# shz9/viprs

Measured on AMD Instinct MI355X. Metric: SNP-updates/sec/E-step (1M SNPs, ~1700 LD blocks), higher is better.
Workload: dtype f32

## Files before the change

### viprs_amd/csrc/estep_grid_mfma.h

```cpp
#pragma once
#include "device_math.h"
#include "kernels_common.h"

namespace viprs {

#ifdef VIPRS_GRID_PROFILE
#define GPROF(slot, cond) do { if (blk == 0 && lane == 0 && p < 32 && (cond)) s_prof[p][slot] = (unsigned)wall_clock64(); } while (0)
#else
#define GPROF(slot, cond) do { } while (0)
#endif

constexpr int kGridIoPitch = kPanel + 1;
constexpr int kGridIoArr = kGridModels * kGridIoPitch;
constexpr int kGridIoFloats = 4 * kGridIoArr;
constexpr int kGridAFloats = kPanel * kGridModels;
constexpr int kGridDiagFloats = kPanel * kPanel;
constexpr int kGridCarryFloats = (kPanel + 32) * 64;
constexpr int kGridQxPitch = kPanel + 4;
constexpr int kGridQxFloats = kGridModels * kGridQxPitch;
constexpr int kGridLdsFloats = 2 * kGridIoFloats + 2 * kGridAFloats + 2 * kGridDiagFloats + kGridCarryFloats + 2 * kGridQxFloats;

using f32x16 = __attribute__((ext_vector_type(16))) float;
using f32x4 = __attribute__((ext_vector_type(4))) float;
using f32x2 = __attribute__((ext_vector_type(2))) float;


template <typename U>
__device__ __forceinline__ void tile_load_rows(float (&R)[kPanel], const U* __restrict__ base, int stride, int b,
                                               int rp, int ct, int lane) {
    const int row0 = rp * kPanel;
    const int last_row = min(kPanel, b - row0) - 1;
    const U* __restrict__ p = base + (int64_t)row0 * stride + ct * kPanel + lane;
#pragma unroll
    for (int k = 0; k < kPanel; ++k) R[k] = static_cast<float>(p[(int64_t)min(k, last_row) * stride]);
    asm volatile("" ::: "memory");
}

template <bool SCALED = false>
__device__ __forceinline__ void tile_compute(f32x16& acc0, f32x16& acc1, const float (&R)[kPanel],
                                             const float* __restrict__ a_lds, int lane, float scale = 1.0f) {
    const int half = lane >> 5, l31 = lane & 31;
#pragma unroll
    for (int kr = 0; kr < kPanel; kr += 2) {
        auto sw = __builtin_amdgcn_permlane32_swap(__float_as_uint(R[kr]), __float_as_uint(R[kr + 1]), false, false);
        const float b0 = __uint_as_float(sw[0]), b1 = __uint_as_float(sw[1]);
        const float a_raw = a_lds[(kr + half) * kGridModels + l31];
        const float aop = SCALED ? scale * a_raw : a_raw;
        acc0 = __builtin_amdgcn_mfma_f32_32x32x2f32(aop, b0, acc0, 0, 0, 0);
        acc1 = __builtin_amdgcn_mfma_f32_32x32x2f32(aop, b1, acc1, 0, 0, 0);
    }
}

template <typename U> struct Vec4 { typedef U type __attribute__((ext_vector_type(4))); };
typedef float f32x4u __attribute__((ext_vector_type(4), aligned(4)));

template <bool FULL>
__device__ __forceinline__ void wtile_load_acc_issue(f32x16 (&acc)[4], const EStepArgs<float>& A, const int* act, int64_t s0,
                                                     int b, int c0, bool lane_ok, int lane) {
    const int half = lane >> 5, c = c0 + 4 * (lane & 31);
#pragma unroll
    for (int r = 0; r < 16; ++r) {
        const int g = (r & 3) + 8 * (r >> 2) + 4 * half;
        const unsigned off = (unsigned)act[g] * (unsigned)A.m + (unsigned)s0;
        if (FULL) {
            const f32x4u v = *reinterpret_cast<const f32x4u*>(A.q + off + (lane_ok ? c : 0));
#pragma unroll
            for (int j = 0; j < 4; ++j) acc[j][r] = v[j];
        } else {
#pragma unroll
            for (int j = 0; j < 4; ++j) acc[j][r] = A.q[off + ((lane_ok && c + j < b) ? c + j : 0)];
        }
    }
    asm volatile("" ::: "memory");
}
template <bool FULL>
__device__ __forceinline__ void wtile_load_acc_finish(f32x16 (&acc)[4], int b, int c0, bool lane_ok, int n_models, int lane) {
    const int half = lane >> 5, c = c0 + 4 * (lane & 31);
#pragma unroll
    for (int r = 0; r < 16; ++r) {
        const int g = (r & 3) + 8 * (r >> 2) + 4 * half;
        const bool ok = lane_ok && g < n_models;
#pragma unroll
        for (int j = 0; j < 4; ++j) acc[j][r] = (ok && (FULL || c + j < b)) ? acc[j][r] : 0.0f;
    }
}
template <bool FULL>
__device__ __forceinline__ void wtile_load_acc(f32x16 (&acc)[4], const EStepArgs<float>& A, const int* act, int64_t s0,
                                               int b, int c0, bool lane_ok, int n_models, int lane) {
    wtile_load_acc_issue<FULL>(acc, A, act, s0, b, c0, lane_ok, lane);
    wtile_load_acc_finish<FULL>(acc, b, c0, lane_ok, n_models, lane);
}

template <bool FULL>
__device__ __forceinline__ void wtile_store_acc(const f32x16 (&acc)[4], const EStepArgs<float>& A, const int* act,
                                                int64_t s0, int b, int c0, bool lane_ok, int n_models, int lane) {
    const int half = lane >> 5, c = c0 + 4 * (lane & 31);
#pragma unroll
    for (int r = 0; r < 16; ++r) {
        const int g = (r & 3) + 8 * (r >> 2) + 4 * half;
        if (lane_ok && g < n_models) {
            const unsigned off = (unsigned)act[g] * (unsigned)A.m + (unsigned)s0 + c;
            if (FULL) {
                *reinterpret_cast<f32x4u*>(A.q + off) = f32x4u{acc[0][r], acc[1][r], acc[2][r], acc[3][r]};
            } else {
#pragma unroll
                for (int j = 0; j < 4; ++j)
                    if (c + j < b) A.q[off + j] = acc[j][r];
            }
        }
    }
}

template <bool FULL>
__device__ __forceinline__ void wtile_add_to_q(const f32x16 (&acc)[4], const EStepArgs<float>& A, const int* act, int64_t s0,
                                               int b, int c0, bool lane_ok, int n_models, int lane, float dq) {
    const int half = lane >> 5, c = c0 + 4 * (lane & 31);
#pragma unroll
    for (int r = 0; r < 16; ++r) {
        const int g = (r & 3) + 8 * (r >> 2) + 4 * half;
        if (lane_ok && g < n_models) {
            const unsigned off = (unsigned)act[g] * (unsigned)A.m + (unsigned)s0 + c;
            if (FULL) {
                const f32x4u v = *reinterpret_cast<const f32x4u*>(A.q + off);
                *reinterpret_cast<f32x4u*>(A.q + off) =
                    f32x4u{v[0] + dq * acc[0][r], v[1] + dq * acc[1][r], v[2] + dq * acc[2][r], v[3] + dq * acc[3][r]};
            } else {
#pragma unroll
                for (int j = 0; j < 4; ++j)
                    if (c + j < b) A.q[off + j] = A.q[off + j] + dq * acc[j][r];
            }
        }
    }
}

template <bool SYM, bool EXACT = true, bool STORE_D = false>
__device__ __forceinline__ void grid_chain_panel(const EStepArgs<float>& A, float* io, float* la, float* dg, float* qx, int p, int b,
                                                 int64_t s0, int lane, int n_models, float dq, const ExpTab& tab
#ifdef VIPRS_GRID_PROFILE
                                                 , int blk, unsigned* prof
#endif
                                                 ) {
    const int cg = lane & 31, ch = lane >> 5;
    const bool has_model = cg < n_models;
#ifdef VIPRS_GRID_PROFILE
    unsigned (*s_prof)[12] = reinterpret_cast<unsigned (*)[12]>(prof);
#endif
    const int r0 = p * kPanel;
    const int nrows = min(kPanel, b - r0);
    float* iob = io + (p & 1) * kGridIoFloats + cg * kGridIoPitch;
    float* lap = la + (p & 1) * kGridAFloats + cg;
    const float* drow = dg + (p & 1) * kGridDiagFloats + 32 * ch;
    float* qmine = qx + (p & 1) * kGridQxFloats + cg * kGridQxPitch + 32 * ch;
    f32x2 qv[16];
#pragma unroll
    for (int i = 0; i < 8; ++i) {
        const f32x4 v = *reinterpret_cast<const f32x4*>(qmine + 4 * i);
        qv[2 * i] = has_model ? f32x2{v[0], v[1]} : f32x2{0.0f, 0.0f};
        qv[2 * i + 1] = has_model ? f32x2{v[2], v[3]} : f32x2{0.0f, 0.0f};
    }
    const float betav = A.std_beta[s0 + min(r0 + lane, b - 1)];
#ifdef VIPRS_GRID_PROFILE
    asm volatile("s_waitcnt vmcnt(0) lgkmcnt(0)" ::: "memory");
#endif
    GPROF(2, true);
    f32x2 rw[16];
    auto load_row = [&](f32x2 (&dst)[16], int jr, int g4) {
        const float* rp = drow + jr * kPanel;
        const int o0 = 16 * (g4 & 1), o1 = 16 * ((g4 + 1) & 1);
#pragma unroll
        for (int i = 0; i < 4; ++i) {
            const f32x4 x = *reinterpret_cast<const f32x4*>(rp + o0 + 4 * i);
            const f32x4 y = *reinterpret_cast<const f32x4*>(rp + o1 + 4 * i);
            dst[2 * i] = f32x2{x[0], x[1]};
            dst[2 * i + 1] = f32x2{x[2], x[3]};
            dst[8 + 2 * i] = f32x2{y[0], y[1]};
            dst[8 + 2 * i + 1] = f32x2{y[2], y[3]};
        }
    };
    load_row(rw, 0, 0);
    float mm = iob[0 * kGridIoArr], ulog = iob[1 * kGridIoArr], hvt = iob[2 * kGridIoArr],
          eta_old = iob[3 * kGridIoArr];
#pragma unroll 1
    for (int g4 = 0; g4 < kPanel / 16; ++g4) {
        const bool hi_owner = g4 >= 2;
        const bool owner = (ch == 1) == hi_owner;
        float* const iog = iob + 16 * g4;
        float* const lag = lap + 16 * g4 * kGridModels;
#pragma unroll
        for (int k = 0; k < 16; ++k) {
            const int jj = 16 * g4 + k;
            const bool live = jj < nrows;
            const int jn = min(jj + 1, kPanel - 1);
            const int kn = (k < 15) ? k + 1 : ((g4 < kPanel / 16 - 1) ? 16 : 15);
            const float mm_n = iog[0 * kGridIoArr + kn], ulog_n = iog[1 * kGridIoArr + kn],
                        hvt_n = iog[2 * kGridIoArr + kn], eta_n = iog[3 * kGridIoArr + kn];
            const unsigned qbits = __float_as_uint(qv[k >> 1][k & 1]);
            auto sw = __builtin_amdgcn_permlane32_swap(qbits, qbits, false, false);
            const float qcur = __uint_as_float(hi_owner ? sw[1] : sw[0]);
            const float beta = __builtin_bit_cast(float, __builtin_amdgcn_readlane(__builtin_bit_cast(int, betav), jj));
            const float mu = mm * (beta - qcur);
            const float u = ulog + hvt * mu * mu;
            const float gamma = EXACT ? sigmoid_exact<kLookupPerLane>(u, tab) : sigmoid_fast(u);
            const float d = gamma * mu - eta_old;
            const float a = (live && has_model) ? dq * d : 0.0f;
            f32x2 rn[16];
            load_row(rn, jn, (jj + 1) >> 4);
            const f32x2 a2 = {a, a};
#pragma unroll
            for (int c = 0; c < 16; ++c) {
                qv[c] = __builtin_elementwise_fma(rw[c], a2, qv[c]);
                asm volatile("" : "+v"(qv[c]));
            }
            if (SYM) qv[k >> 1][k & 1] -= (live && owner && has_model) ? d : 0.0f;
            iog[0 * kGridIoArr + k] = mu;
            iog[1 * kGridIoArr + k] = gamma;
            iog[2 * kGridIoArr + k] = d;
            iog[3 * kGridIoArr + k] = eta_old + d;
            lag[k * kGridModels] = STORE_D ? ((live && has_model) ? d : 0.0f) : a;
            mm = mm_n; ulog = ulog_n; hvt = hvt_n; eta_old = eta_n;
#pragma unroll
            for (int c = 0; c < 16; ++c) rw[c] = rn[c];
            __builtin_amdgcn_sched_barrier(0);
        }
#pragma unroll
        for (int c = 0; c < 8; ++c) {
            const f32x2 t = qv[c];
            qv[c] = qv[8 + c];
            qv[8 + c] = t;
        }
    }
    GPROF(3, true);
    if (has_model) {
#pragma unroll
        for (int i = 0; i < 8; ++i)
            *reinterpret_cast<f32x4*>(qmine + 4 * i) = f32x4{qv[2 * i][0], qv[2 * i][1], qv[2 * i + 1][0], qv[2 * i + 1][1]};
    }
}

template <bool SYM, bool EXACT = true>
__device__ __forceinline__ void grid_chain_panel_mfma(const EStepArgs<float>& A, float* io, float* la, float* dg, float* qx, int p,
                                                      int b, int64_t s0, int lane, int n_models, float dq, const ExpTab& tab) {
    const int cg = lane & 31, ch = lane >> 5;
    const bool has_model = cg < n_models;
    const int r0 = p * kPanel;
    const int nrows = min(kPanel, b - r0);
    float* iob = io + (p & 1) * kGridIoFloats + cg * kGridIoPitch;
    float* lap = la + (p & 1) * kGridAFloats + cg;
    const float* drow = dg + (p & 1) * kGridDiagFloats + lane;
    float* qm = qx + (p & 1) * kGridQxFloats + cg * kGridQxPitch;
    f32x16 acc0, acc1;
#pragma unroll
    for (int g = 0; g < 4; ++g) {
        const f32x4 v = *reinterpret_cast<const f32x4*>(qm + 8 * g + 4 * ch);
        const f32x4 w = *reinterpret_cast<const f32x4*>(qm + 32 + 8 * g + 4 * ch);
#pragma unroll
        for (int e = 0; e < 4; ++e) {
            acc0[4 * g + e] = has_model ? v[e] : 0.0f;
            acc1[4 * g + e] = has_model ? w[e] : 0.0f;
        }
    }
    const float betav = A.std_beta[s0 + min(r0 + lane, b - 1)];
    float mm = iob[0 * kGridIoArr], ulog = iob[1 * kGridIoArr], hvt = iob[2 * kGridIoArr], eta_old = iob[3 * kGridIoArr];
    float rowv = drow[0];
    float qcur;
    {
        const unsigned x = __float_as_uint(acc0[0]);
        auto sx = __builtin_amdgcn_permlane32_swap(x, x, false, false);
        qcur = __uint_as_float(sx[0]);
    }
#pragma unroll
    for (int jj = 0; jj < kPanel; ++jj) {
        const bool live = jj < nrows;
        const int jn = (jj + 1 < kPanel) ? jj + 1 : jj;
        const float mm_n = iob[0 * kGridIoArr + jn], ulog_n = iob[1 * kGridIoArr + jn], hvt_n = iob[2 * kGridIoArr + jn],
                    eta_n = iob[3 * kGridIoArr + jn];
        const float rowv_n = drow[jn * kPanel];
        const float beta = __builtin_bit_cast(float, __builtin_amdgcn_readlane(__builtin_bit_cast(int, betav), jj));
        const float mu = mm * (beta - qcur);
        const float u = ulog + hvt * mu * mu;
        const float gamma = EXACT ? sigmoid_exact<kLookupPerLane>(u, tab) : sigmoid_fast(u);
        const float d = gamma * mu - eta_old;
        const float a = (live && has_model) ? dq * d : 0.0f;
        const float dsub = (SYM && live && has_model) ? d : 0.0f;
        __builtin_amdgcn_sched_barrier(0);
        auto sr = __builtin_amdgcn_permlane32_swap(__float_as_uint(rowv), __float_as_uint(rowv), false, false);
        const float row_lo = __uint_as_float(sr[0]), row_hi = __uint_as_float(sr[1]);
        const float A0 = ch ? ((SYM && cg == jj) ? -1.0f : 0.0f) : row_lo;
        const float A1 = ch ? ((SYM && cg + 32 == jj) ? -1.0f : 0.0f) : row_hi;
        const float B = ch ? dsub : a;
        float qnext = 0.0f;
        if (jj + 1 < kPanel) {
            constexpr int kDummy = 0; (void)kDummy;
            const int c1 = jj + 1, i1 = c1 & 31, r1 = (i1 & 3) + 4 * (i1 >> 3), h1 = (i1 >> 2) & 1;
            const unsigned x = __float_as_uint((c1 >> 5) ? acc1[r1] : acc0[r1]);
            auto sx = __builtin_amdgcn_permlane32_swap(x, x, false, false);
            const float xq = __uint_as_float(h1 ? sx[1] : sx[0]);
            const float dn = __builtin_bit_cast(float, __builtin_amdgcn_readlane(__builtin_bit_cast(int, rowv), c1));
            qnext = __builtin_fmaf(dn, a, xq);
        }
        acc0 = __builtin_amdgcn_mfma_f32_32x32x2f32(A0, B, acc0, 0, 0, 0);
        acc1 = __builtin_amdgcn_mfma_f32_32x32x2f32(A1, B, acc1, 0, 0, 0);
        if (has_model && live && ch == 0) {
            iob[0 * kGridIoArr + jj] = mu;
            iob[1 * kGridIoArr + jj] = gamma;
            iob[2 * kGridIoArr + jj] = d;
            iob[3 * kGridIoArr + jj] = eta_old + d;
        }
        if (ch == 0) lap[jj * kGridModels] = a;
        mm = mm_n; ulog = ulog_n; hvt = hvt_n; eta_old = eta_n; rowv = rowv_n; qcur = qnext;
        __builtin_amdgcn_sched_barrier(0);
    }
    if (has_model) {
#pragma unroll
        for (int g = 0; g < 4; ++g) {
            *reinterpret_cast<f32x4*>(qm + 8 * g + 4 * ch) = f32x4{acc0[4 * g], acc0[4 * g + 1], acc0[4 * g + 2], acc0[4 * g + 3]};
            *reinterpret_cast<f32x4*>(qm + 32 + 8 * g + 4 * ch) = f32x4{acc1[4 * g], acc1[4 * g + 1], acc1[4 * g + 2], acc1[4 * g + 3]};
        }
    }
}

constexpr int kGridWaves = 8;
constexpr int kGridNU = kGridWaves - 1;
constexpr int kGridPerWave = (kGridModels + kGridNU - 1) / kGridNU;
constexpr int kGridDiagPerWave = (kPanel + kGridNU - 1) / kGridNU;


constexpr int kGridCarryWave = 4;


template <typename U> struct RawCols4;
template <> struct RawCols4<float> {
    f32x4 v;
    static constexpr int kDwords = 4;
    __device__ __forceinline__ void mask(bool on) { v = on ? v : f32x4{0.0f, 0.0f, 0.0f, 0.0f}; }
    __device__ __forceinline__ void mask_below(int row, int col0) {
#pragma unroll
        for (int j = 0; j < 4; ++j) v[j] = row > col0 + j ? v[j] : 0.0f;
    }
    template <int J> __device__ __forceinline__ float get() const { return v[J]; }
};
template <> struct RawCols4<int8_t> {
    unsigned w;
    static constexpr int kDwords = 1;
    __device__ __forceinline__ void mask(bool on) { w = on ? w : 0u; }
    __device__ __forceinline__ void mask_below(int row, int col0) {
        unsigned m = 0u;
#pragma unroll
        for (int j = 0; j < 4; ++j) m |= row > col0 + j ? 0xFFu << (8 * j) : 0u;
        w &= m;
    }
    template <int J> __device__ __forceinline__ float get() const { return static_cast<float>(static_cast<int8_t>(w >> (8 * J))); }
};
template <> struct RawCols4<int16_t> {
    unsigned w[2];
    static constexpr int kDwords = 2;
    __device__ __forceinline__ void mask(bool on) { w[0] = on ? w[0] : 0u; w[1] = on ? w[1] : 0u; }
    __device__ __forceinline__ void mask_below(int row, int col0) {
#pragma unroll
        for (int h = 0; h < 2; ++h) {
            const unsigned m = (row > col0 + 2 * h ? 0xFFFFu : 0u) | (row > col0 + 2 * h + 1 ? 0xFFFF0000u : 0u);
            w[h] &= m;
        }
    }
    template <int J> __device__ __forceinline__ float get() const { return static_cast<float>(static_cast<int16_t>(w[J >> 1] >> (16 * (J & 1)))); }
};
template <typename U> __device__ __forceinline__ RawCols4<U> load_cols4(const char* p);
template <> __device__ __forceinline__ RawCols4<float> load_cols4<float>(const char* p) {
    return RawCols4<float>{*reinterpret_cast<const f32x4*>(p)};
}
template <> __device__ __forceinline__ RawCols4<int8_t> load_cols4<int8_t>(const char* p) {
    return RawCols4<int8_t>{*reinterpret_cast<const unsigned*>(p)};
}
template <> __device__ __forceinline__ RawCols4<int16_t> load_cols4<int16_t>(const char* p) {
    const uint2 t = *reinterpret_cast<const uint2*>(p);
    return RawCols4<int16_t>{{t.x, t.y}};
}
template <typename U, bool MIRV = false>
__device__ __forceinline__ void res_tile_apply(f32x16 (&acc)[4], const U* __restrict__ base, int stride, int pp, int c0,
                                               int lane, bool on_l, bool on_r, const float* __restrict__ a_lds,
                                               float scale = 1.0f, int tri = -1) {
    const int half = lane >> 5, l31 = lane & 31;
    const bool lane_on = (lane & 16) ? on_r : on_l;
    const bool lane_tri = MIRV && tri >= 0 && ((lane & 16) != 0) == (tri == 1);
    int tri_col0 = 4 * (l31 & 15);
    if (MIRV) asm volatile("" : "+v"(tri_col0));
    int col = c0 + 4 * l31;
    if (col >= stride) col = c0;
    const unsigned voff = (unsigned)((half * stride + (col - c0)) * (int)sizeof(U));
    const char* __restrict__ sb = reinterpret_cast<const char*>(base + (int64_t)pp * kPanel * stride + c0);
    const size_t step = (size_t)2 * stride * sizeof(U);
    constexpr int CH = 8 * 4 / RawCols4<U>::kDwords, NCH = kPanel / 2 / CH;
    RawCols4<U> ring[CH];
#pragma unroll
    for (int c = 0; c < NCH; ++c) {
#pragma unroll
        for (int i = 0; i < CH; ++i) ring[i] = load_cols4<U>(sb + (c * CH + i) * step + voff);
        asm volatile("" ::: "memory");
#pragma unroll
        for (int i = 0; i < CH; ++i) {
            RawCols4<U> v = ring[i];
            v.mask(lane_on);
            if (MIRV && tri >= 0) { if (lane_tri) v.mask_below(2 * (c * CH + i) + half, tri_col0); }
            const float a_raw = a_lds[(2 * (c * CH + i) + half) * kGridModels + l31];
            const float aop = MIRV ? scale * a_raw : a_raw;
            acc[0] = __builtin_amdgcn_mfma_f32_32x32x2f32(aop, v.template get<0>(), acc[0], 0, 0, 0);
            acc[1] = __builtin_amdgcn_mfma_f32_32x32x2f32(aop, v.template get<1>(), acc[1], 0, 0, 0);
            acc[2] = __builtin_amdgcn_mfma_f32_32x32x2f32(aop, v.template get<2>(), acc[2], 0, 0, 0);
            acc[3] = __builtin_amdgcn_mfma_f32_32x32x2f32(aop, v.template get<3>(), acc[3], 0, 0, 0);
        }
    }
}

struct GridTeam {
    int member = 0, size = 1;
    unsigned long long* gran = nullptr;
    uint32_t tag_base = 0;
};
constexpr int kGridTeamPanels = 2 * kGridResOwners * kGridResSlots;

template <typename U, bool SYM, bool EXACT>
__device__ __forceinline__ void grid_block_resident(const EStepArgs<float>& A, float* io, float* la, float* dg, f32x4* cy,
                                                    float* qx, const int* s_act, const BlockDesc& bd, int wave, int lane,
                                                    int n_models, float dq, const ExpTab& tab, const GridTeam tm = GridTeam()) {
    constexpr bool MIR = !SYM;
    constexpr int NU = kGridNU;
    const int64_t s0 = bd.start;
    const int b = bd.size, stride = bd.stride;
    const U* __restrict__ base = static_cast<const U*>(A.ld_dense) + bd.ld_off;
    const int np = (b + kPanel - 1) / kPanel;
    float* cq = reinterpret_cast<float*>(cy + 16 * 64);
    const int half = lane >> 5, n = lane & 31;
    const bool team = tm.size > 1;
    const int p_lo = tm.member * kGridTeamPanels, p_hi = min(np, p_lo + kGridTeamPanels);
    const int T_lo = tm.member * kGridResOwners * kGridResSlots;
    auto mine = [&](int p) { return !team || (p >= p_lo && p < p_hi); };
    const int p_end = np;
    auto publish_a = [&](int p) {
        const float* src = la + (p & 1) * kGridAFloats;
        unsigned long long* g = tm.gran + (int64_t)p * kGridAFloats;
        const unsigned long long tag = (unsigned long long)(tm.tag_base + (unsigned)(p + 1)) << 32;
#pragma unroll 8
        for (int i = 0; i < kGridAFloats / 64; ++i)
            __hip_atomic_store(g + i * 64 + lane, tag | (unsigned long long)__float_as_uint(src[i * 64 + lane]), __ATOMIC_RELAXED,
                               __HIP_MEMORY_SCOPE_AGENT);
    };
    auto receive_a = [&](int p) {
        float* dst = la + (p & 1) * kGridAFloats;
        const unsigned long long* g = tm.gran + (int64_t)p * kGridAFloats;
        const unsigned want = tm.tag_base + (unsigned)(p + 1);
        for (int i0 = 0; i0 < kGridAFloats / 64; i0 += 8) {
            unsigned long long v[8];
            for (unsigned spins = 0;; ++spins) {
                bool ok = true;
#pragma unroll
                for (int k = 0; k < 8; ++k) {
                    v[k] = __hip_atomic_load(g + (i0 + k) * 64 + lane, __ATOMIC_RELAXED, __HIP_MEMORY_SCOPE_AGENT);
                    ok = ok && (unsigned)(v[k] >> 32) == want;
                }
                if (__all(ok)) break;
                if (spins > (1u << 22)) {
                    if (lane == 0) atomicExch(A.error, 1);
                    break;
                }
                if ((spins & 255u) == 0u && __hip_atomic_load(A.error, __ATOMIC_RELAXED, __HIP_MEMORY_SCOPE_AGENT) != 0) break;
                __builtin_amdgcn_s_sleep(16);
            }
#pragma unroll
            for (int k = 0; k < 8; ++k) dst[(i0 + k) * 64 + lane] = __uint_as_float((unsigned)v[k]);
        }
    };

    auto stage_inputs = [&](int pp, bool with_q) {
        float* dst = io + (pp & 1) * kGridIoFloats;
        const int r0 = pp * kPanel;
        const int j = r0 + lane;
        const bool ok = j < b;
        const unsigned jo = (unsigned)s0 + (ok ? j : 0);
        float v[kGridPerWave][5];
#pragma unroll
        for (int i = 0; i < kGridPerWave; ++i) {
            const int g = min(wave - 1 + NU * i, kGridModels - 1);
            const unsigned off = (unsigned)s_act[g] * (unsigned)A.m + jo;
            v[i][0] = A.mu_mult[off]; v[i][1] = A.u_logs[off]; v[i][2] = A.shvt[off]; v[i][3] = A.eta[off];
            v[i][4] = with_q ? A.q[off] : 0.0f;
        }
        const int nrows = min(kPanel, b - r0);
        const U* __restrict__ dp = base + (int64_t)r0 * stride + r0 + lane;
        float dv[kGridDiagPerWave];
#pragma unroll
        for (int i = 0; i < kGridDiagPerWave; ++i)
            dv[i] = static_cast<float>(dp[(int64_t)min(wave - 1 + NU * i, nrows - 1) * stride]);
        asm volatile("" ::: "memory");
#pragma unroll
        for (int i = 0; i < kGridPerWave; ++i) {
            const int g = wave - 1 + NU * i;
            if (g < n_models) {
#pragma unroll
                for (int a = 0; a < 4; ++a) dst[a * kGridIoArr + g * kGridIoPitch + lane] = ok ? v[i][a] : 0.0f;
                if (with_q) qx[(pp & 1) * kGridQxFloats + g * kGridQxPitch + lane] = ok ? v[i][4] : 0.0f;
            }
        }
        float* dd = dg + (pp & 1) * kGridDiagFloats;
#pragma unroll
        for (int i = 0; i < kGridDiagPerWave; ++i) {
            const int t = wave - 1 + NU * i;
            if (t < kPanel) dd[t * kPanel + lane] = (MIR && lane <= t) ? 0.0f : dv[i];
        }
    };
    auto flush_outputs = [&](int pp) {
        const float* src = io + (pp & 1) * kGridIoFloats;
        const float* qs = qx + (pp & 1) * kGridQxFloats;
        const int j = pp * kPanel + lane;
        if (j < b) {
#pragma unroll
            for (int i = 0; i < kGridPerWave; ++i) {
                const int g = wave - 1 + NU * i;
                if (g < n_models) {
                    const unsigned off = (unsigned)s_act[g] * (unsigned)A.m + (unsigned)(s0 + j);
                    A.var_mu[off] = src[0 * kGridIoArr + g * kGridIoPitch + lane];
                    A.var_gamma[off] = src[1 * kGridIoArr + g * kGridIoPitch + lane];
                    A.eta_diff[off] = src[2 * kGridIoArr + g * kGridIoPitch + lane];
                    A.eta[off] = src[3 * kGridIoArr + g * kGridIoPitch + lane];
                    if (!SYM) A.q[off] = qs[g * kGridQxPitch + lane];
                }
            }
        }
    };

    if (wave == 0) {
        __syncthreads();
        for (int p = 0; p <= p_end; ++p) {
            __syncthreads();
            if (p < np && mine(p)) {
#ifdef VIPRS_GRID_MFMA_CHAIN
                grid_chain_panel_mfma<SYM, EXACT>(A, io, la, dg, qx, p, b, s0, lane, n_models, dq, tab);
#else
                grid_chain_panel<SYM, EXACT, MIR>(A, io, la, dg, qx, p, b, s0, lane, n_models, dq, tab
#ifdef VIPRS_GRID_PROFILE
                                      , 1, nullptr
#endif
                                      );
#endif
            } else if (p < np) {
                receive_a(p);
            }
            __syncthreads();
        }
    } else if (wave == kGridCarryWave) {
        if (mine(0)) stage_inputs(0, true);
        __syncthreads();
        f32x16 c0v, c1v;
#pragma unroll
        for (int r = 0; r < 16; ++r) { c0v[r] = 0.0f; c1v[r] = 0.0f; }
        for (int p = 0; p <= p_end; ++p) {
            if (p > 0 && p < np && mine(p)) {
                float R1[kPanel];
#pragma unroll
                for (int i = 0; i < 16; ++i) {
                    const f32x4 v = cy[i * 64 + lane];
#pragma unroll
                    for (int e = 0; e < 4; ++e) R1[4 * i + e] = v[e];
                }
                tile_compute<MIR>(c0v, c1v, R1, la + ((p - 1) & 1) * kGridAFloats, lane, dq);
                float* qd = qx + (p & 1) * kGridQxFloats + n;
#pragma unroll
                for (int r = 0; r < 16; ++r) {
                    const int g = (r & 3) + 8 * (r >> 2) + 4 * half;
                    qd[g * kGridQxPitch] = c0v[r];
                    qd[g * kGridQxPitch + 32] = c1v[r];
                }
            }
            if (p + 1 < np && mine(p + 1)) {
#pragma unroll
                for (int r = 0; r < 16; ++r) {
                    const int g = (r & 3) + 8 * (r >> 2) + 4 * half;
                    c0v[r] = cq[g * kPanel + n];
                    c1v[r] = cq[g * kPanel + 32 + n];
                }
            }
            __syncthreads();
            if (team && p > 0 && mine(p - 1)) publish_a(p - 1);
            if (p > 0 && mine(p - 1)) flush_outputs(p - 1);
            if (p + 1 < np && mine(p + 1)) stage_inputs(p + 1, false);
            if (p + 1 < np && mine(p + 1)) {
                if (p > 0) {
                    float R0[kPanel];
                    tile_load_rows<U>(R0, base, stride, b, p - 1, p + 1, lane);
                    tile_compute<MIR>(c0v, c1v, R0, la + ((p - 1) & 1) * kGridAFloats, lane, dq);
                    asm volatile("" : "+v"(c0v), "+v"(c1v) :: "memory");
                }
                float R1[kPanel];
                tile_load_rows<U>(R1, base, stride, b, p, p + 1, lane);
#pragma unroll
                for (int i = 0; i < 16; ++i) cy[i * 64 + lane] = f32x4{R1[4 * i], R1[4 * i + 1], R1[4 * i + 2], R1[4 * i + 3]};
            }
            __syncthreads();
        }
    } else {
        const int ow = wave < kGridCarryWave ? wave - 1 : wave - 2;
        f32x16 accA[4], accB[4];
        const int TA = T_lo + ow, TB = T_lo + ow + kGridResOwners;
        const int cA = TA * 2 * kPanel, cB = TB * 2 * kPanel;
        const bool hasA = cA < b, hasB = cB < b;
        auto load_tile = [&](f32x16 (&acc)[4], int c0, bool has) {
            if (!has) {
#pragma unroll
                for (int j = 0; j < 4; ++j)
#pragma unroll
                    for (int r = 0; r < 16; ++r) acc[j][r] = 0.0f;
                return;
            }
            const bool lane_ok = (n < 16) || (c0 + kPanel < b);
            if (c0 + 2 * kPanel <= b) wtile_load_acc<true>(acc, A, s_act, s0, b, c0, lane_ok, n_models, lane);
            else wtile_load_acc<false>(acc, A, s_act, s0, b, c0, lane_ok, n_models, lane);
        };
        load_tile(accA, cA, hasA);
        load_tile(accB, cB, hasB);
        auto extract = [&](const f32x16 (&acc)[4], int e) {
            if ((n >= 16) == ((e & 1) != 0)) {
#pragma unroll
                for (int r = 0; r < 16; ++r) {
                    const int g = (r & 3) + 8 * (r >> 2) + 4 * half;
                    *reinterpret_cast<f32x4*>(cq + g * kPanel + 4 * (n & 15)) = f32x4{acc[0][r], acc[1][r], acc[2][r], acc[3][r]};
                }
            }
        };
        auto take_back = [&](f32x16 (&acc)[4], int e) {
            if ((n >= 16) == ((e & 1) != 0)) {
                const float* qs = qx + (e & 1) * kGridQxFloats;
#pragma unroll
                for (int r = 0; r < 16; ++r) {
                    const int g = (r & 3) + 8 * (r >> 2) + 4 * half;
                    const f32x4 v = *reinterpret_cast<const f32x4*>(qs + g * kGridQxPitch + 4 * (n & 15));
                    const bool okg = g < n_models;
#pragma unroll
                    for (int j = 0; j < 4; ++j) acc[j][r] = okg ? v[j] : 0.0f;
                }
            }
        };
        auto restart = [&](f32x16 (&acc)[4], int e) {
            if ((n >= 16) == ((e & 1) != 0)) {
#pragma unroll
                for (int j = 0; j < 4; ++j)
#pragma unroll
                    for (int r = 0; r < 16; ++r) acc[j][r] = 0.0f;
            }
        };
        auto tile_of = [&](int panel) { return panel >> 1; };
        if (np > 1) {
            if (tile_of(1) == TA) extract(accA, 1);
        }
        if (mine(0)) stage_inputs(0, true);
        __syncthreads();
        for (int p = 0; p <= p_end; ++p) {
            __syncthreads();
            if (p > 0 && mine(p - 1)) flush_outputs(p - 1);
            if (p + 1 < np && mine(p + 1)) stage_inputs(p + 1, false);
            if (p > 0) {
                const int pp = p - 1;
                if (SYM) {
                    if (tile_of(pp) == TA) take_back(accA, pp);
                    else if (tile_of(pp) == TB) take_back(accB, pp);
                }
                if (MIR) {
                    if (tile_of(pp) == TA) restart(accA, pp);
                    else if (tile_of(pp) == TB) restart(accB, pp);
                }
                const float* a_lds = la + (pp & 1) * kGridAFloats;
                auto panel_on = [&](int c) {
                    if (c >= np) return false;
                    return c < p - 1 || c > p + 1 || (MIR && c == p - 1);
                };
                auto apply = [&](f32x16 (&acc)[4], int T, int c0) {
                    const bool l = panel_on(2 * T), r = panel_on(2 * T + 1);
                    if (!(l || r)) return;
                    if constexpr (MIR) {
                        const int tri = 2 * T == pp ? 0 : (2 * T + 1 == pp ? 1 : -1);
                        res_tile_apply<U, true>(acc, base, stride, pp, c0, lane, l, r, a_lds, 2 * T <= pp ? 1.0f : dq, tri);
                    } else {
                        res_tile_apply<U>(acc, base, stride, pp, c0, lane, l, r, a_lds);
                    }
                };
                if (hasA) apply(accA, TA, cA);
                if (hasB) apply(accB, TB, cB);
            }
            if (p + 2 < np) {
                const int e = p + 2;
                if (tile_of(e) == TA) extract(accA, e);
                else if (tile_of(e) == TB) extract(accB, e);
            }
            __syncthreads();
        }
        if (MIR) {
            auto add_tile = [&](const f32x16 (&acc)[4], int c0) {
                const bool lane_ok = (n < 16) || (c0 + kPanel < b);
                if (c0 + 2 * kPanel <= b) wtile_add_to_q<true>(acc, A, s_act, s0, b, c0, lane_ok, n_models, lane, dq);
                else wtile_add_to_q<false>(acc, A, s_act, s0, b, c0, lane_ok, n_models, lane, dq);
            };
            if (hasA) add_tile(accA, cA);
            if (hasB) add_tile(accB, cB);
        }
        if (SYM) {
            auto store_tile = [&](const f32x16 (&acc)[4], int c0) {
                const bool lane_ok = (n < 16) || (c0 + kPanel < b);
                if (c0 + 2 * kPanel <= b) wtile_store_acc<true>(acc, A, s_act, s0, b, c0, lane_ok, n_models, lane);
                else wtile_store_acc<false>(acc, A, s_act, s0, b, c0, lane_ok, n_models, lane);
            };
            if (hasA) store_tile(accA, cA);
            if (hasB) store_tile(accB, cB);
        }
    }
}

struct GridTeams {
    int32_t n_wgs = 0, n_blocks = 0;
    int32_t queue_start = 0;
    const int32_t* block = nullptr;
    const int32_t* member = nullptr;
    const int32_t* size = nullptr;
    const int64_t* goff = nullptr;
    unsigned long long* gran = nullptr;
    uint32_t tag_base = 0;
};

__device__ __forceinline__ int grid_group_models(const int32_t* __restrict__ blk_group, const int32_t* __restrict__ lists,
                                                 int* s_act, int blk, int tid) {
    const int32_t* __restrict__ l = lists + (int64_t)__builtin_amdgcn_readfirstlane(blk_group[__builtin_amdgcn_readfirstlane(blk)]) *
                                                kGroupListStride;
    if (tid < kGridModels) s_act[tid] = l[1 + tid];
    const int cnt = __builtin_amdgcn_readfirstlane(l[0]);
    __syncthreads();
    return cnt;
}

template <typename U, bool SYM, bool EXACT, bool GROUPED = false>
__global__ __launch_bounds__(64 * kGridWaves) void estep_grid_mfma_kernel(EStepArgs<float> A, GridTeams teams) {
    extern __shared__ __attribute__((aligned(16))) float smem[];
    float* io = smem;
    float* la = smem + 2 * kGridIoFloats;
    float* dg = la + 2 * kGridAFloats;
    f32x4* cy = reinterpret_cast<f32x4*>(dg + 2 * kGridDiagFloats);
    float* qx = dg + 2 * kGridDiagFloats + kGridCarryFloats;
    __shared__ int s_blk;
    __shared__ int s_act[kGridModels];
    const int tid = threadIdx.x;
    const int wave = __builtin_amdgcn_readfirstlane(tid >> 6);
    const int lane = tid & 63;
    const int n_models = A.n_active;
    const float dq = A.dq;
    ExpTab tab;
    tab.init();
    if (tid < kGridModels) s_act[tid] = A.active[min(tid, n_models - 1)];
    __syncthreads();

    if ((int)blockIdx.x < teams.n_wgs) {
        const int tb = teams.block[blockIdx.x];
        GridTeam tm;
        tm.member = teams.member[blockIdx.x];
        tm.size = teams.size[blockIdx.x];
        tm.gran = teams.gran + teams.goff[tb];
        tm.tag_base = teams.tag_base;
        if constexpr (GROUPED) {
            const int nm = grid_group_models(A.blk_group, A.group_lists, s_act, tb, tid);
            if (nm > 0) grid_block_resident<U, SYM, EXACT>(A, io, la, dg, cy, qx, s_act, A.blocks[tb], wave, lane, nm, dq, tab, tm);
        } else {
            grid_block_resident<U, SYM, EXACT>(A, io, la, dg, cy, qx, s_act, A.blocks[tb], wave, lane, n_models, dq, tab, tm);
        }
        __syncthreads();
    }
    for (;;) {
        if (tid == 0) s_blk = teams.queue_start + atomicAdd(A.counter, 1);
        __syncthreads();
        const int blk = s_blk;
        __syncthreads();
        if (blk >= A.n_blocks) break;
        const BlockDesc bd = A.blocks[blk];
        if (bd.size > kGridResMaxCols) {
            __hip_atomic_store(A.error, 2, __ATOMIC_RELAXED, __HIP_MEMORY_SCOPE_AGENT);
            continue;
        }
        if constexpr (GROUPED) {
            const int nm = grid_group_models(A.blk_group, A.group_lists, s_act, blk, tid);
            if (nm > 0) grid_block_resident<U, SYM, EXACT>(A, io, la, dg, cy, qx, s_act, bd, wave, lane, nm, dq, tab);
            continue;
        }
        grid_block_resident<U, SYM, EXACT>(A, io, la, dg, cy, qx, s_act, bd, wave, lane, n_models, dq, tab);
    }
}

}
```

### viprs_amd/csrc/kernels_common.h

```cpp
#pragma once
#include <hip/hip_runtime.h>
#include <stdint.h>

#if (defined(PANEL_TIMING_NO_HANDOFF_WAIT) || \
    defined(PANEL_TIMING_NO_SECOND_PASS) || \
    defined(PANEL_NW) || \
    defined(PANEL_STRIP_DEPTH) || \
    defined(PANEL_MIN_WAVES) || \
    defined(PANEL_TEAM_STRIP_DEPTH) || \
    defined(PANEL_TEAM_CPL_F32) || \
    defined(PANEL_CHAIN_PRIO) || \
    defined(VIPRS_LD_STREAM) || \
    defined(VIPRS_LD_STREAM_PARTIAL) || \
    defined(VIPRS_LD_STREAM_NARROW) || \
    defined(VIPRS_GRID_MFMA_CHAIN) || \
    defined(VIPRS_GRID_PROFILE) || \
    defined(VIPRS_TILE_PROFILE) || \
    defined(VIPRS_SWEEP_TRACE) || \
    defined(VIPRS_PANEL_PROFILE)) && \
    !defined(VIPRS_EXPERIMENTAL)
#error "experiment switch defined without -DVIPRS_EXPERIMENTAL (see kernels_common.h)"
#endif
#ifdef VIPRS_EXPERIMENTAL
#define VIPRS_BF_VIPRS_EXPERIMENTAL " VIPRS_EXPERIMENTAL"
#else
#define VIPRS_BF_VIPRS_EXPERIMENTAL ""
#endif
#ifdef PANEL_TIMING_NO_HANDOFF_WAIT
#define VIPRS_BF_PANEL_TIMING_NO_HANDOFF_WAIT " PANEL_TIMING_NO_HANDOFF_WAIT"
#else
#define VIPRS_BF_PANEL_TIMING_NO_HANDOFF_WAIT ""
#endif
#ifdef PANEL_TIMING_NO_SECOND_PASS
#define VIPRS_BF_PANEL_TIMING_NO_SECOND_PASS " PANEL_TIMING_NO_SECOND_PASS"
#else
#define VIPRS_BF_PANEL_TIMING_NO_SECOND_PASS ""
#endif
#ifdef PANEL_NW
#define VIPRS_BF_PANEL_NW " PANEL_NW"
#else
#define VIPRS_BF_PANEL_NW ""
#endif
#ifdef PANEL_STRIP_DEPTH
#define VIPRS_BF_PANEL_STRIP_DEPTH " PANEL_STRIP_DEPTH"
#else
#define VIPRS_BF_PANEL_STRIP_DEPTH ""
#endif
#ifdef PANEL_MIN_WAVES
#define VIPRS_BF_PANEL_MIN_WAVES " PANEL_MIN_WAVES"
#else
#define VIPRS_BF_PANEL_MIN_WAVES ""
#endif
#ifdef PANEL_TEAM_STRIP_DEPTH
#define VIPRS_BF_PANEL_TEAM_STRIP_DEPTH " PANEL_TEAM_STRIP_DEPTH"
#else
#define VIPRS_BF_PANEL_TEAM_STRIP_DEPTH ""
#endif
#ifdef PANEL_TEAM_CPL_F32
#define VIPRS_BF_PANEL_TEAM_CPL_F32 " PANEL_TEAM_CPL_F32"
#else
#define VIPRS_BF_PANEL_TEAM_CPL_F32 ""
#endif
#ifdef PANEL_CHAIN_PRIO
#define VIPRS_BF_PANEL_CHAIN_PRIO " PANEL_CHAIN_PRIO"
#else
#define VIPRS_BF_PANEL_CHAIN_PRIO ""
#endif
#ifdef VIPRS_LD_STREAM
#define VIPRS_BF_VIPRS_LD_STREAM " VIPRS_LD_STREAM"
#else
#define VIPRS_BF_VIPRS_LD_STREAM ""
#endif
#ifdef VIPRS_LD_STREAM_PARTIAL
#define VIPRS_BF_VIPRS_LD_STREAM_PARTIAL " VIPRS_LD_STREAM_PARTIAL"
#else
#define VIPRS_BF_VIPRS_LD_STREAM_PARTIAL ""
#endif
#ifdef VIPRS_LD_STREAM_NARROW
#define VIPRS_BF_VIPRS_LD_STREAM_NARROW " VIPRS_LD_STREAM_NARROW"
#else
#define VIPRS_BF_VIPRS_LD_STREAM_NARROW ""
#endif
#ifdef VIPRS_GRID_MFMA_CHAIN
#define VIPRS_BF_VIPRS_GRID_MFMA_CHAIN " VIPRS_GRID_MFMA_CHAIN"
#else
#define VIPRS_BF_VIPRS_GRID_MFMA_CHAIN ""
#endif
#ifdef VIPRS_GRID_PROFILE
#define VIPRS_BF_VIPRS_GRID_PROFILE " VIPRS_GRID_PROFILE"
#else
#define VIPRS_BF_VIPRS_GRID_PROFILE ""
#endif
#ifdef VIPRS_TILE_PROFILE
#define VIPRS_BF_VIPRS_TILE_PROFILE " VIPRS_TILE_PROFILE"
#else
#define VIPRS_BF_VIPRS_TILE_PROFILE ""
#endif
#ifdef VIPRS_SWEEP_TRACE
#define VIPRS_BF_VIPRS_SWEEP_TRACE " VIPRS_SWEEP_TRACE"
#else
#define VIPRS_BF_VIPRS_SWEEP_TRACE ""
#endif
#ifdef VIPRS_PANEL_PROFILE
#define VIPRS_BF_VIPRS_PANEL_PROFILE " VIPRS_PANEL_PROFILE"
#else
#define VIPRS_BF_VIPRS_PANEL_PROFILE ""
#endif
#define VIPRS_TU_BUILD_FLAGS VIPRS_BF_VIPRS_EXPERIMENTAL VIPRS_BF_PANEL_TIMING_NO_HANDOFF_WAIT VIPRS_BF_PANEL_TIMING_NO_SECOND_PASS VIPRS_BF_PANEL_NW VIPRS_BF_PANEL_STRIP_DEPTH VIPRS_BF_PANEL_MIN_WAVES VIPRS_BF_PANEL_TEAM_STRIP_DEPTH VIPRS_BF_PANEL_TEAM_CPL_F32 VIPRS_BF_PANEL_CHAIN_PRIO VIPRS_BF_VIPRS_LD_STREAM VIPRS_BF_VIPRS_LD_STREAM_PARTIAL VIPRS_BF_VIPRS_LD_STREAM_NARROW VIPRS_BF_VIPRS_GRID_MFMA_CHAIN VIPRS_BF_VIPRS_GRID_PROFILE VIPRS_BF_VIPRS_TILE_PROFILE VIPRS_BF_VIPRS_SWEEP_TRACE VIPRS_BF_VIPRS_PANEL_PROFILE

namespace viprs {
void register_build_flags(const char* flags);
struct BuildFlagsRegistrar { explicit BuildFlagsRegistrar(const char* f) { register_build_flags(f); } };
}

namespace viprs {

constexpr int kPanel = 64;
constexpr int kStrip = 256;

constexpr int kPanelMaxK = 8;
constexpr int kPanelWideMaxK = 31;
constexpr int kMixLdsFloats = 5 * kPanel * kPanelMaxK;
struct PanelLds {
    int qcap;
    bool mix_scratch, mirror;
    __host__ __device__ constexpr PanelLds(int qcap_, bool mix_scratch_, bool mirror_)
        : qcap(qcap_), mix_scratch(mix_scratch_), mirror(mirror_) {}
    __host__ __device__ constexpr int q() const { return 0; }
    __host__ __device__ constexpr int a() const { return qcap; }
    __host__ __device__ constexpr int diag_tiles() const { return a() + 2 * kPanel; }
    __host__ __device__ constexpr int offdiag_tile() const { return diag_tiles() + 2 * kPanel * kPanel; }
    __host__ __device__ constexpr int mix() const { return offdiag_tile() + kPanel * kPanel; }
    __host__ __device__ constexpr int ed() const { return mix() + (mix_scratch ? kMixLdsFloats : 0); }
    __host__ __device__ constexpr int s() const { return ed() + 2 * kPanel; }
    __host__ __device__ constexpr int total_floats() const { return mirror ? s() + qcap : ed(); }
};
constexpr int kMaxMixtureK = 64;
constexpr int kGridModels = 32;
constexpr int kGridResOwners = 6, kGridResSlots = 2;
constexpr int kGridResMaxCols = kGridResOwners * kGridResSlots * 2 * kPanel;
constexpr int kBandMaxRingPanels = 256;

struct BlockDesc {
    int32_t start;
    int32_t size;
    int32_t stride;
    int32_t kind;
    int64_t ld_off;
    int64_t gr_off;
    int32_t band_left;
    int32_t band_right;
};

template <typename T>
struct EStepArgs {
    const BlockDesc* blocks;
    int32_t n_blocks;
    int32_t* counter;
    int32_t bottom_mod;
    unsigned long long* granules;
    uint32_t tag_base;
    int32_t* arrive;
    int32_t* error;
    int32_t n_teams;
    int32_t team_size;
    int64_t granule_rows;
    unsigned long long* skipped;
    const int32_t* lb;
    const int64_t* rowstart;
    const int32_t* rowlen;
    const void* ld_rows;
    const void* ld_dense;
    int64_t ld_zero_off;
    const T* std_beta;
    const T* u_logs;
    const T* shvt;
    const T* mu_mult;
    const T* log_null_pi;
    T* var_gamma;
    T* var_mu;
    T* eta;
    T* q;
    T* eta_diff;
    T* eta_out;
    T* q_out;
    T dq;
    int32_t low_memory;
    int32_t width;
    int64_t m;
    const int32_t* active;
    int32_t n_active;
    const int32_t* blk_group;
    const uint8_t* group_cols;
    const int32_t* group_lists;
};
constexpr int kGroupListStride = 1 + kGridModels;

template <typename T>
__device__ __forceinline__ EStepArgs<T> select_model(const EStepArgs<T>& A0, int model_slot) {
    EStepArgs<T> A = A0;
    if (A0.n_active > 0) {
        const int64_t off = (int64_t)A0.active[model_slot] * A0.m;
        A.var_gamma += off; A.var_mu += off; A.eta += off; A.q += off; A.eta_diff += off;
        A.u_logs += off; A.shvt += off; A.mu_mult += off;
        if (A.eta_out) { A.eta_out += off; A.q_out += off; }
    }
    return A;
}

}
```

Measured before the change: 1.680 billion.

## Overlap carry-wave tile compute with chain wave via LDS progress counter

The chain wave now publishes a per-16-row progress counter in shared memory. The carry wave uses it to start its MFMA carry update on the rows already finalized for the next panel, instead of waiting for the whole panel at the barrier. Only the last 16-row group is left after the sync. This shortens the serial critical path per panel. In exchange it adds spin-wait polling with s_sleep, a volatile LDS flag, and ordering that relies only on compiler barriers, so there is a risk of memory-ordering races and of polling overhead.

```diff
diff --git a/viprs_amd/csrc/estep_grid_mfma.h b/viprs_amd/csrc/estep_grid_mfma.h
--- a/viprs_amd/csrc/estep_grid_mfma.h
+++ b/viprs_amd/csrc/estep_grid_mfma.h
@@ -1,6 +1,14 @@
 #pragma once
 #include "device_math.h"
 #include "kernels_common.h"
+
+#ifndef VIPRS_GRID_CARRY_OVERLAP
+#ifdef VIPRS_GRID_MFMA_CHAIN
+#define VIPRS_GRID_CARRY_OVERLAP 0
+#else
+#define VIPRS_GRID_CARRY_OVERLAP 1
+#endif
+#endif
 
 namespace viprs {
 
@@ -51,6 +59,30 @@
     }
 }
 
+template <bool SCALED>
+__device__ __forceinline__ void tile_compute_rows16(f32x16& acc0, f32x16& acc1, const f32x4* __restrict__ tile,
+                                                    const float* __restrict__ a_lds, int g, int lane, float scale) {
+    const int half = lane >> 5, l31 = lane & 31;
+    const f32x4* __restrict__ tg = tile + 4 * g * 64 + lane;
+    const float* __restrict__ ag = a_lds + (16 * g + half) * kGridModels + l31;
+    float R[16];
+#pragma unroll
+    for (int i = 0; i < 4; ++i) {
+        const f32x4 v = tg[i * 64];
+#pragma unroll
+        for (int e = 0; e < 4; ++e) R[4 * i + e] = v[e];
+    }
+#pragma unroll
+    for (int kr = 0; kr < 16; kr += 2) {
+        auto sw = __builtin_amdgcn_permlane32_swap(__float_as_uint(R[kr]), __float_as_uint(R[kr + 1]), false, false);
+        const float b0 = __uint_as_float(sw[0]), b1 = __uint_as_float(sw[1]);
+        const float a_raw = ag[kr * kGridModels];
+        const float aop = SCALED ? scale * a_raw : a_raw;
+        acc0 = __builtin_amdgcn_mfma_f32_32x32x2f32(aop, b0, acc0, 0, 0, 0);
+        acc1 = __builtin_amdgcn_mfma_f32_32x32x2f32(aop, b1, acc1, 0, 0, 0);
+    }
+}
+
 template <typename U> struct Vec4 { typedef U type __attribute__((ext_vector_type(4))); };
 typedef float f32x4u __attribute__((ext_vector_type(4), aligned(4)));
 
@@ -135,7 +167,8 @@
 
 template <bool SYM, bool EXACT = true, bool STORE_D = false>
 __device__ __forceinline__ void grid_chain_panel(const EStepArgs<float>& A, float* io, float* la, float* dg, float* qx, int p, int b,
-                                                 int64_t s0, int lane, int n_models, float dq, const ExpTab& tab
+                                                 int64_t s0, int lane, int n_models, float dq, const ExpTab& tab,
+                                                 int* progress
 #ifdef VIPRS_GRID_PROFILE
                                                  , int blk, unsigned* prof
 #endif
@@ -228,6 +261,10 @@
             qv[c] = qv[8 + c];
             qv[8 + c] = t;
         }
+#if VIPRS_GRID_CARRY_OVERLAP
+        asm volatile("" ::: "memory");
+        if (lane == 0) *reinterpret_cast<volatile int*>(progress) = kPanel * p + 16 * (g4 + 1);
+#endif
     }
     GPROF(3, true);
     if (has_model) {
@@ -421,7 +458,8 @@
 template <typename U, bool SYM, bool EXACT>
 __device__ __forceinline__ void grid_block_resident(const EStepArgs<float>& A, float* io, float* la, float* dg, f32x4* cy,
                                                     float* qx, const int* s_act, const BlockDesc& bd, int wave, int lane,
-                                                    int n_models, float dq, const ExpTab& tab, const GridTeam tm = GridTeam()) {
+                                                    int n_models, float dq, const ExpTab& tab, int* progress,
+                                                    const GridTeam tm = GridTeam()) {
     constexpr bool MIR = !SYM;
     constexpr int NU = kGridNU;
     const int64_t s0 = bd.start;
@@ -535,7 +573,7 @@
 #ifdef VIPRS_GRID_MFMA_CHAIN
                 grid_chain_panel_mfma<SYM, EXACT>(A, io, la, dg, qx, p, b, s0, lane, n_models, dq, tab);
 #else
-                grid_chain_panel<SYM, EXACT, MIR>(A, io, la, dg, qx, p, b, s0, lane, n_models, dq, tab
+                grid_chain_panel<SYM, EXACT, MIR>(A, io, la, dg, qx, p, b, s0, lane, n_models, dq, tab, progress
 #ifdef VIPRS_GRID_PROFILE
                                       , 1, nullptr
 #endif
@@ -548,12 +586,33 @@
         }
     } else if (wave == kGridCarryWave) {
         if (mine(0)) stage_inputs(0, true);
+#if VIPRS_GRID_CARRY_OVERLAP
+        if (lane == 0) *reinterpret_cast<volatile int*>(progress) = 0;
+#endif
         __syncthreads();
         f32x16 c0v, c1v;
 #pragma unroll
         for (int r = 0; r < 16; ++r) { c0v[r] = 0.0f; c1v[r] = 0.0f; }
+#if VIPRS_GRID_CARRY_OVERLAP
+        auto wait_rows = [&](int want) {
+            for (unsigned spins = 0; *reinterpret_cast<volatile int*>(progress) < want; ++spins) {
+                if (spins > (1u << 18)) {
+                    if (lane == 0) atomicExch(A.error, 1);
+                    break;
+                }
+                __builtin_amdgcn_s_sleep(8);
+            }
+            asm volatile("" ::: "memory");
+        };
+#endif
         for (int p = 0; p <= p_end; ++p) {
             if (p > 0 && p < np && mine(p)) {
+#if VIPRS_GRID_CARRY_OVERLAP
+                const float* ap = la + ((p - 1) & 1) * kGridAFloats;
+#pragma unroll 1
+                for (int g = mine(p - 1) ? 3 : 0; g < 4; ++g)
+                    tile_compute_rows16<MIR>(c0v, c1v, cy, ap, g, lane, dq);
+#else
                 float R1[kPanel];
 #pragma unroll
                 for (int i = 0; i < 16; ++i) {
@@ -562,6 +621,7 @@
                     for (int e = 0; e < 4; ++e) R1[4 * i + e] = v[e];
                 }
                 tile_compute<MIR>(c0v, c1v, R1, la + ((p - 1) & 1) * kGridAFloats, lane, dq);
+#endif
                 float* qd = qx + (p & 1) * kGridQxFloats + n;
 #pragma unroll
                 for (int r = 0; r < 16; ++r) {
@@ -594,6 +654,16 @@
 #pragma unroll
                 for (int i = 0; i < 16; ++i) cy[i * 64 + lane] = f32x4{R1[4 * i], R1[4 * i + 1], R1[4 * i + 2], R1[4 * i + 3]};
             }
+#if VIPRS_GRID_CARRY_OVERLAP
+            if (p + 1 < np && mine(p + 1) && mine(p)) {
+                const float* ap = la + (p & 1) * kGridAFloats;
+#pragma unroll 1
+                for (int g = 0; g < 3; ++g) {
+                    wait_rows(kPanel * p + 16 * (g + 1));
+                    tile_compute_rows16<MIR>(c0v, c1v, cy, ap, g, lane, dq);
+                }
+            }
+#endif
             __syncthreads();
         }
     } else {
@@ -743,6 +813,12 @@
     float* qx = dg + 2 * kGridDiagFloats + kGridCarryFloats;
     __shared__ int s_blk;
     __shared__ int s_act[kGridModels];
+#if VIPRS_GRID_CARRY_OVERLAP
+    __shared__ int s_progress;
+    int* progress = &s_progress;
+#else
+    int* progress = nullptr;
+#endif
     const int tid = threadIdx.x;
     const int wave = __builtin_amdgcn_readfirstlane(tid >> 6);
     const int lane = tid & 63;
@@ -762,9 +838,9 @@
         tm.tag_base = teams.tag_base;
         if constexpr (GROUPED) {
             const int nm = grid_group_models(A.blk_group, A.group_lists, s_act, tb, tid);
-            if (nm > 0) grid_block_resident<U, SYM, EXACT>(A, io, la, dg, cy, qx, s_act, A.blocks[tb], wave, lane, nm, dq, tab, tm);
+            if (nm > 0) grid_block_resident<U, SYM, EXACT>(A, io, la, dg, cy, qx, s_act, A.blocks[tb], wave, lane, nm, dq, tab, progress, tm);
         } else {
-            grid_block_resident<U, SYM, EXACT>(A, io, la, dg, cy, qx, s_act, A.blocks[tb], wave, lane, n_models, dq, tab, tm);
+            grid_block_resident<U, SYM, EXACT>(A, io, la, dg, cy, qx, s_act, A.blocks[tb], wave, lane, n_models, dq, tab, progress, tm);
         }
         __syncthreads();
     }
@@ -781,11 +857,11 @@
         }
         if constexpr (GROUPED) {
             const int nm = grid_group_models(A.blk_group, A.group_lists, s_act, blk, tid);
-            if (nm > 0) grid_block_resident<U, SYM, EXACT>(A, io, la, dg, cy, qx, s_act, bd, wave, lane, nm, dq, tab);
+            if (nm > 0) grid_block_resident<U, SYM, EXACT>(A, io, la, dg, cy, qx, s_act, bd, wave, lane, nm, dq, tab, progress);
             continue;
         }
-        grid_block_resident<U, SYM, EXACT>(A, io, la, dg, cy, qx, s_act, bd, wave, lane, n_models, dq, tab);
-    }
-}
-
-}
+        grid_block_resident<U, SYM, EXACT>(A, io, la, dg, cy, qx, s_act, bd, wave, lane, n_models, dq, tab, progress);
+    }
+}
+
+}
diff --git a/viprs_amd/csrc/kernels_common.h b/viprs_amd/csrc/kernels_common.h
--- a/viprs_amd/csrc/kernels_common.h
+++ b/viprs_amd/csrc/kernels_common.h
@@ -15,6 +15,7 @@
     defined(VIPRS_LD_STREAM_NARROW) || \
     defined(VIPRS_GRID_MFMA_CHAIN) || \
     defined(VIPRS_GRID_PROFILE) || \
+    defined(VIPRS_GRID_CARRY_OVERLAP) || \
     defined(VIPRS_TILE_PROFILE) || \
     defined(VIPRS_SWEEP_TRACE) || \
     defined(VIPRS_PANEL_PROFILE)) && \
@@ -91,6 +92,11 @@
 #else
 #define VIPRS_BF_VIPRS_GRID_PROFILE ""
 #endif
+#ifdef VIPRS_GRID_CARRY_OVERLAP
+#define VIPRS_BF_VIPRS_GRID_CARRY_OVERLAP " VIPRS_GRID_CARRY_OVERLAP"
+#else
+#define VIPRS_BF_VIPRS_GRID_CARRY_OVERLAP ""
+#endif
 #ifdef VIPRS_TILE_PROFILE
 #define VIPRS_BF_VIPRS_TILE_PROFILE " VIPRS_TILE_PROFILE"
 #else
@@ -106,7 +112,7 @@
 #else
 #define VIPRS_BF_VIPRS_PANEL_PROFILE ""
 #endif
-#define VIPRS_TU_BUILD_FLAGS VIPRS_BF_VIPRS_EXPERIMENTAL VIPRS_BF_PANEL_TIMING_NO_HANDOFF_WAIT VIPRS_BF_PANEL_TIMING_NO_SECOND_PASS VIPRS_BF_PANEL_NW VIPRS_BF_PANEL_STRIP_DEPTH VIPRS_BF_PANEL_MIN_WAVES VIPRS_BF_PANEL_TEAM_STRIP_DEPTH VIPRS_BF_PANEL_TEAM_CPL_F32 VIPRS_BF_PANEL_CHAIN_PRIO VIPRS_BF_VIPRS_LD_STREAM VIPRS_BF_VIPRS_LD_STREAM_PARTIAL VIPRS_BF_VIPRS_LD_STREAM_NARROW VIPRS_BF_VIPRS_GRID_MFMA_CHAIN VIPRS_BF_VIPRS_GRID_PROFILE VIPRS_BF_VIPRS_TILE_PROFILE VIPRS_BF_VIPRS_SWEEP_TRACE VIPRS_BF_VIPRS_PANEL_PROFILE
+#define VIPRS_TU_BUILD_FLAGS VIPRS_BF_VIPRS_EXPERIMENTAL VIPRS_BF_PANEL_TIMING_NO_HANDOFF_WAIT VIPRS_BF_PANEL_TIMING_NO_SECOND_PASS VIPRS_BF_PANEL_NW VIPRS_BF_PANEL_STRIP_DEPTH VIPRS_BF_PANEL_MIN_WAVES VIPRS_BF_PANEL_TEAM_STRIP_DEPTH VIPRS_BF_PANEL_TEAM_CPL_F32 VIPRS_BF_PANEL_CHAIN_PRIO VIPRS_BF_VIPRS_LD_STREAM VIPRS_BF_VIPRS_LD_STREAM_PARTIAL VIPRS_BF_VIPRS_LD_STREAM_NARROW VIPRS_BF_VIPRS_GRID_MFMA_CHAIN VIPRS_BF_VIPRS_GRID_PROFILE VIPRS_BF_VIPRS_GRID_CARRY_OVERLAP VIPRS_BF_VIPRS_TILE_PROFILE VIPRS_BF_VIPRS_SWEEP_TRACE VIPRS_BF_VIPRS_PANEL_PROFILE
 
 namespace viprs {
 void register_build_flags(const char* flags);
```

Result: no change. 1.677 billion (-0.2%).
